# bruniss/multi-task-3d-resencoder-unet

Hardware: AMD Instinct MI355X
Metric: train patches/sec (b,c,z,y,x) ResEncM 1x128^3 (higher is better)
Workload: dtype bf16; 1 GPU; cfg2: ResEncM (6 stages, feats [32, 64, 128, 256, 512, 512], blocks [1, 3, 4, 6, 6, 6]), 1-in, heads ['sheet'], patch 128x128x128, batch 2/GPU, full train step (fwd+loss+bwd+allreduce+clip+AdamW); global_batch=2, parallelism=dp1

## Files before the change

multi-task-3d-resencoder-unet_amd/csrc/build.py:

```python
import os
import subprocess
import sys

HERE = os.path.dirname(os.path.abspath(__file__))
SOURCES = ["rx_runtime.hip", "rx_instnorm.hip", "rx_head.hip", "rx_stem.hip", "rx_pack_optim.hip", "rx_igemm.hip", "rx_wgrad.hip", "rx_wgrad_halo.hip", "rx_conv_halo.hip", "rx_stem_wgrad.hip", "rx_loss.hip", "rx_se.hip", "rx_dgrad_s2.hip", "rx_prog.hip", "rx_pointwise.hip", "rx_infer.hip", "rx_augment.hip", "rx_geometry.hip"]
HEADERS = ["rx_common.h", "rx_internal.h", "rx_reduce.h", "rx_prog.h", os.path.join("..", "..", "include", "rxunet.h")]
LIB = os.path.join(HERE, "librxunet.so")
HIPCC = os.environ.get("HIPCC", "/opt/rocm/bin/hipcc")
FLAGS = ["-O3", "--offload-arch=gfx950", "-std=c++17", "-fPIC", "-Wno-unused-result"]


def _stale(target, deps):
    if not os.path.exists(target):
        return True
    t = os.path.getmtime(target)
    return any(os.path.getmtime(d) > t for d in deps)


def build(force=False, verbose=True):
    hdrs = [os.path.join(HERE, h) for h in HEADERS] + [os.path.abspath(__file__)]
    objs = []
    procs = []
    for src in SOURCES:
        obj = os.path.join(HERE, src.replace(".hip", ".o"))
        objs.append(obj)
        if force or _stale(obj, [os.path.join(HERE, src)] + hdrs):
            cmd = [HIPCC] + FLAGS + ["-c", os.path.join(HERE, src), "-o", obj]
            if verbose:
                print(" ".join(cmd), flush=True)
            procs.append((src, subprocess.Popen(cmd, cwd=HERE)))
    for src, p in procs:
        if p.wait() != 0:
            raise RuntimeError(f"hipcc failed on {src}")
    if force or procs or _stale(LIB, objs):
        cmd = [HIPCC, "--offload-arch=gfx950", "-shared", "-fPIC", "-o", LIB] + objs
        if verbose:
            print(" ".join(cmd), flush=True)
        subprocess.check_call(cmd, cwd=HERE)
    return LIB


if __name__ == "__main__":
    print(build(force="--force" in sys.argv))
```

multi-task-3d-resencoder-unet_amd/csrc/rx_internal.h:

```cpp
#pragma once
#include "rx_common.h"

int rx_note_seq(void);

int rx_conv_halo_try(rx_dtype dt, const rx_act* in, const void* w, const float* bias, const rx_act* out, int flip, int accumulate,
                     hipStream_t st, float* stat_part, size_t stat_bytes, int* stat_chunks, const RxBwdStat* bs);
int rx_pointwise_try(rx_dtype dt, const rx_act* in, const void* w, const float* bias, const rx_act* out, const int32_t stride[3],
                     int accumulate, hipStream_t st);
int rx_dgrad_s2_halo_try(rx_dtype dt, const rx_act* dy, const void* w_bwd, const rx_act* dx, int accumulate, hipStream_t st);

size_t rx_wgrad_halo_ws_bytes(const rx_act* x, const rx_act* dy);
int rx_wgrad_halo_try(rx_dtype dt, const rx_act* x, const rx_act* dy, const int32_t stride[3], float* dw, void* ws, size_t ws_bytes,
                      hipStream_t st);
void rx_wgrad_reduce_launch(const float* slab, int S, int T_, int R, int C, float* dw, hipStream_t st);

int rx_stem_fwd_mfma_try(rx_dtype dt, const float* x, int n, int cin, int z, int y, int xx, const float* w, const float* bias,
                         const rx_act* out, const int32_t kernel[3], hipStream_t st, float* stat_part, size_t stat_bytes, int* stat_chunks);
int rx_stem_wgrad_mfma_try(rx_dtype dt, const float* x, int n, int cin, int z, int y, int xx, const rx_act* dy, const int32_t kernel[3],
                           float* partial, int max_blocks, int* nblocks_out, hipStream_t st);

void rx_colreduce_finalize_launch(hipStream_t st, const float* partial, int N, int nchunks, int nacc, int C, double V, float eps, int mode,
                                  float* out);
void rx_stats_finalize_launch(const float* partial, int N, int nchunks, int C, double V, float eps, float* stats, hipStream_t st);
void rx_inbwd_fused_finalize_launch(const float* partial, int N, int nchunks, int C, double V, const float* stats, float* m12, hipStream_t st);
```

multi-task-3d-resencoder-unet_amd/csrc/rx_wgrad.hip:

```cpp
#include <stdlib.h>

#include "rx_common.h"
#include "rx_internal.h"


struct WgradGeom {
  int Qz, Qy, Qx, Vq, NQ;
  int R, ldg;
  long g_ss;
  int Zx, Yx, Xx, Cc, ldx;
  long x_ss;
  int isz, isy, isx;
  int ntaps, ksplit, q_per_split, tiles_c;
  RxTap taps[RX_MAX_TAPS];
};


typedef __attribute__((address_space(3))) s16x4 lds_s16x4;

template <typename T>
__device__ inline u32x4 fetch_frag(const T* panel, int ks, int lane) {
  if constexpr (sizeof(T) == 2) {
    const int g16 = lane >> 4, half = g16 & 1, h = g16 >> 1, l15 = lane & 15, q4 = l15 >> 2, p4 = l15 & 3;
    const T* a0 = panel + (ks * 16 + 8 * h + q4) * 32 + 16 * half + 4 * p4;
    s16x4 t0 = __builtin_amdgcn_ds_read_tr16_b64_v4i16((lds_s16x4*)(a0));
    s16x4 t1 = __builtin_amdgcn_ds_read_tr16_b64_v4i16((lds_s16x4*)(a0 + 4 * 32));
    u32x2 lo = __builtin_bit_cast(u32x2, t0), hi = __builtin_bit_cast(u32x2, t1);
    return u32x4{lo[0], lo[1], hi[0], hi[1]};
  } else {
    const int i = lane & 31, h = lane >> 5;
    const T* a0 = panel + (ks * 8 + 4 * h) * 32 + i;
    f32x4 v = {a0[0], a0[32], a0[64], a0[96]};
    return __builtin_bit_cast(u32x4, v);
  }
}

template <typename T, int BR, int BC>
__global__ __launch_bounds__(256) void wgrad_kernel(const T* __restrict__ gt, const T* __restrict__ xt, float* __restrict__ slab,
                                                    const WgradGeom g) {
  constexpr int P = Elem<T>::PER16;
  constexpr int NR = BR / 32, NC = BC / 32;
  constexpr int GV = 64 * BR / P / 256;
  constexpr int XV = 64 * BC / P / 256;
  constexpr int KSTEPS = sizeof(T) == 2 ? 4 : 8;
  constexpr int TILE_ELEMS = 64 * (BR + BC);
  extern __shared__ __attribute__((aligned(16))) unsigned char smem[];
  T* sbuf = reinterpret_cast<T*>(smem);

  const int tid = threadIdx.x, lane = tid & 63, wave = tid >> 6;
  const int tile_r = blockIdx.x / g.tiles_c, tile_c = blockIdx.x - tile_r * g.tiles_c;
  const int r0 = tile_r * BR, c0 = tile_c * BC;
  const RxTap tp = g.taps[blockIdx.y];
  const int q_begin = blockIdx.z * g.q_per_split;
  const int q_end = min(g.NQ, q_begin + g.q_per_split);

  u32x4 gr[GV], xr[XV];
  auto load_tile = [&](int q0) {
#pragma unroll
    for (int j = 0; j < GV; ++j) {
      const int i = tid + 256 * j, vox = i / (BR / P), cv = i - vox * (BR / P);
      const int q = q0 + vox;
      u32x4 v = u32x4{0u, 0u, 0u, 0u};
      if (q < q_end) {
        const int n = q / g.Vq, vq = q - n * g.Vq;
        v = *reinterpret_cast<const u32x4*>(gt + n * g.g_ss + (long)vq * g.ldg + r0 + cv * P);
      }
      gr[j] = v;
    }
#pragma unroll
    for (int j = 0; j < XV; ++j) {
      const int i = tid + 256 * j, vox = i / (BC / P), cv = i - vox * (BC / P);
      const int q = q0 + vox;
      u32x4 v = u32x4{0u, 0u, 0u, 0u};
      if (q < q_end) {
        const int n = q / g.Vq, vq = q - n * g.Vq;
        const int qx = vq % g.Qx, t = vq / g.Qx;
        const int qy = t % g.Qy, qz = t / g.Qy;
        const int z = qz * g.isz + tp.dz, y = qy * g.isy + tp.dy, x = qx * g.isx + tp.dx;
        if ((unsigned)z < (unsigned)g.Zx && (unsigned)y < (unsigned)g.Yx && (unsigned)x < (unsigned)g.Xx)
          v = *reinterpret_cast<const u32x4*>(xt + n * g.x_ss + ((long)(z * g.Yx + y) * g.Xx + x) * g.ldx + c0 + cv * P);
      }
      xr[j] = v;
    }
  };
  auto store_tile = [&](int buf) {
    T* base = sbuf + buf * TILE_ELEMS;
#pragma unroll
    for (int j = 0; j < GV; ++j) {
      const int i = tid + 256 * j, vox = i / (BR / P), cv = i - vox * (BR / P);
      const int c = cv * P;
      *reinterpret_cast<u32x4*>(base + ((c >> 5) * 64 + vox) * 32 + (c & 31)) = gr[j];
    }
    T* xb = base + 64 * BR;
#pragma unroll
    for (int j = 0; j < XV; ++j) {
      const int i = tid + 256 * j, vox = i / (BC / P), cv = i - vox * (BC / P);
      const int c = cv * P;
      *reinterpret_cast<u32x4*>(xb + ((c >> 5) * 64 + vox) * 32 + (c & 31)) = xr[j];
    }
  };

  f32x16 acc[NR][NC];
#pragma unroll
  for (int a = 0; a < NR; ++a)
#pragma unroll
    for (int b = 0; b < NC; ++b)
#pragma unroll
      for (int r = 0; r < 16; ++r) acc[a][b][r] = 0.f;

  if (q_begin < q_end) {
    load_tile(q_begin);
    store_tile(0);
  }
  __syncthreads();
  int it = 0;
  for (int q0 = q_begin; q0 < q_end; q0 += 64, ++it) {
    const int buf = it & 1;
    if (q0 + 64 < q_end) load_tile(q0 + 64);
    const T* base = sbuf + buf * TILE_ELEMS;
#pragma unroll
    for (int kk = 0; kk < KSTEPS / 4; ++kk) {
      const int ks = wave + 4 * kk;
      u32x4 af[NR], bf[NC];
#pragma unroll
      for (int a = 0; a < NR; ++a) af[a] = fetch_frag<T>(base + a * 64 * 32, ks, lane);
#pragma unroll
      for (int b = 0; b < NC; ++b) bf[b] = fetch_frag<T>(base + 64 * BR + b * 64 * 32, ks, lane);
#pragma unroll
      for (int a = 0; a < NR; ++a)
#pragma unroll
        for (int b = 0; b < NC; ++b) Mma<T>::run(acc[a][b], af[a], bf[b]);
    }
    if (q0 + 64 < q_end) store_tile(buf ^ 1);
    __syncthreads();
  }

  float* red = reinterpret_cast<float*>(smem);
  const int col = lane & 31, fh = lane >> 5;
#pragma unroll
  for (int a = 0; a < NR; ++a)
#pragma unroll
    for (int b = 0; b < NC; ++b)
#pragma unroll
      for (int r = 0; r < 16; ++r) {
        const int row = (r & 3) + 8 * (r >> 2) + 4 * fh;
        red[(((wave * NR + a) * NC + b) * 32 + row) * 32 + col] = acc[a][b][r];
      }
  __syncthreads();
  float* out = slab + ((long)blockIdx.z * g.ntaps + blockIdx.y) * g.R * g.Cc;
  for (int i = tid; i < NR * NC * 1024; i += 256) {
    const int blk = i >> 10, rc = i & 1023, row = rc >> 5, cc = rc & 31;
    const int a = blk / NC, b = blk - a * NC;
    float s = red[i] + red[i + NR * NC * 1024] + red[i + 2 * NR * NC * 1024] + red[i + 3 * NR * NC * 1024];
    out[(long)(r0 + a * 32 + row) * g.Cc + c0 + b * 32 + cc] = s;
  }
}

__global__ __launch_bounds__(256) void wgrad_reduce(const float* __restrict__ slab, int S, int T_, int R, int C, float* __restrict__ dw) {
  __shared__ float tile[27 * 257];
  const long RC = (long)R * C;
  const long base = (long)blockIdx.x * 256;
  const long i = base + threadIdx.x;
  for (int t = 0; t < T_; ++t) {
    float s = 0.f;
    if (i < RC)
      for (int k = 0; k < S; ++k) s += slab[((long)k * T_ + t) * RC + i];
    tile[t * 257 + threadIdx.x] = s;
  }
  __syncthreads();
  const long n_here = (RC - base < 256 ? RC - base : 256) * T_;
  for (long j = threadIdx.x; j < n_here; j += 256) {
    int pair = (int)(j / T_), t = (int)(j - (long)pair * T_);
    dw[base * T_ + j] = tile[t * 257 + pair];
  }
}

__global__ __launch_bounds__(256) void wgrad_reduce_manysplits(const float* __restrict__ slab, int S, int T_, int R, int C,
                                                               float* __restrict__ dw) {
  const long RC = (long)R * C;
  const long i = (long)blockIdx.x * 256 + threadIdx.x;
  const int t = blockIdx.y;
  if (i >= RC) return;
  const float* p = slab + (long)t * RC + i;
  const long stride = (long)T_ * RC;
  float a0 = 0.f, a1 = 0.f, a2 = 0.f, a3 = 0.f, a4 = 0.f, a5 = 0.f, a6 = 0.f, a7 = 0.f;
  int k = 0;
  for (; k + 8 <= S; k += 8) {
    a0 += p[(k + 0) * stride];
    a1 += p[(k + 1) * stride];
    a2 += p[(k + 2) * stride];
    a3 += p[(k + 3) * stride];
    a4 += p[(k + 4) * stride];
    a5 += p[(k + 5) * stride];
    a6 += p[(k + 6) * stride];
    a7 += p[(k + 7) * stride];
  }
  for (; k < S; ++k) a0 += p[k * stride];
  dw[i * T_ + t] = ((a0 + a1) + (a2 + a3)) + ((a4 + a5) + (a6 + a7));
}

static int plan_split(const WgradGeom& g, int BR, int BC, size_t ws_bytes, int* ksplit, int* qps) {
  const long tiles = (long)(g.R / BR) * (g.Cc / BC) * g.ntaps;
  const long ktiles = ((long)g.NQ + 63) / 64;
  long S = (1024 + tiles - 1) / tiles;
  if (S > ktiles / 4) S = ktiles / 4;
  if (S < 1) S = 1;
  const size_t slab1 = (size_t)g.ntaps * g.R * g.Cc * sizeof(float);
  while (S > 1 && S * slab1 > ws_bytes) --S;
  if (slab1 > ws_bytes) return RX_EWORKSPACE;
  long per = (ktiles + S - 1) / S;
  S = (ktiles + per - 1) / per;
  *ksplit = (int)S;
  *qps = (int)(per * 64);
  return RX_OK;
}

static size_t wgrad_ws_bytes(int R, int C, int taps, long NQ) {
  const size_t slab1 = (size_t)taps * R * C * sizeof(float);
  const long tiles = (long)((R + 63) / 64) * ((C + 63) / 64) * taps;
  long S = (1024 + tiles - 1) / tiles;
  long ktiles = (NQ + 63) / 64;
  if (S > ktiles / 4) S = ktiles / 4;
  if (S < 1) S = 1;
  if (R % 64 || C % 64) {
    const long t32 = (long)(R / 32) * (C / 32) * taps;
    long S2 = (1024 + t32 - 1) / t32;
    if (S2 > S) S = S2;
  }
  return S * slab1 + 256;
}

template <typename T>
static void wgrad_dispatch(int BR, int BC, dim3 grid, hipStream_t st, const void* gt, const void* xt, float* slab, const WgradGeom& g) {
  const size_t lds = 65536;
#define RX_WG(BR_, BC_)                                                                                                            \
  do {                                                                                                                             \
    (void)hipFuncSetAttribute(reinterpret_cast<const void*>(&wgrad_kernel<T, BR_, BC_>), hipFuncAttributeMaxDynamicSharedMemorySize, \
                              (int)lds);                                                                                           \
    hipLaunchKernelGGL((wgrad_kernel<T, BR_, BC_>), grid, dim3(256), lds, st, (const T*)gt, (const T*)xt, slab, g);                \
  } while (0)
  if (BR == 64 && BC == 64)
    RX_WG(64, 64);
  else if (BR == 64 && BC == 32)
    RX_WG(64, 32);
  else if (BR == 32 && BC == 64)
    RX_WG(32, 64);
  else
    RX_WG(32, 32);
#undef RX_WG
}

static int wgrad_launch(rx_dtype dt, const void* gt, const void* xt, float* dw, WgradGeom& g, void* ws, size_t ws_bytes, hipStream_t st) {
  const int per16 = dt == RX_F32 ? 4 : 8;
  if (g.R % 32 || g.Cc % 32) RX_FAIL(RX_EUNSUPPORTED, "wgrad: channel counts must be multiples of 32 (R=%d C=%d)", g.R, g.Cc);
  if (g.ldg % per16 || g.ldx % per16 || ((uintptr_t)gt & 15) || ((uintptr_t)xt & 15)) RX_FAIL(RX_EUNSUPPORTED, "wgrad: misaligned operand");
  if (!ws || !dw) RX_FAIL(RX_EINVAL, "wgrad: null workspace / output");
  const int BR = g.R % 64 == 0 ? 64 : 32, BC = g.Cc % 64 == 0 ? 64 : 32;
  g.tiles_c = g.Cc / BC;
  int rc = plan_split(g, BR, BC, ws_bytes, &g.ksplit, &g.q_per_split);
  if (rc) RX_FAIL(rc, "wgrad: workspace too small (%zu bytes)", ws_bytes);
  dim3 grid((g.R / BR) * (g.Cc / BC), g.ntaps, g.ksplit);
  rx_note_kernel(BR == 64 ? (BC == 64 ? "wgrad_kernel<64,64>" : "wgrad_kernel<64,32>") : (BC == 64 ? "wgrad_kernel<32,64>" : "wgrad_kernel<32,32>"));
  RX_DISPATCH_DTYPE(dt, T, wgrad_dispatch<T>(BR, BC, grid, st, gt, xt, (float*)ws, g));
  rx_wgrad_reduce_launch((const float*)ws, g.ksplit, g.ntaps, g.R, g.Cc, dw, st);
  RX_CHECK_LAUNCH("wgrad");
  return RX_OK;
}

static int conv_out_dim(int in, int k, int s) { return (in + 2 * ((k - 1) / 2) - k) / s + 1; }

void rx_wgrad_reduce_launch(const float* slab, int S, int T_, int R, int C, float* dw, hipStream_t st) {
  long RC = (long)R * C;
  if (S >= 8 || T_ > 27)
    hipLaunchKernelGGL(wgrad_reduce_manysplits, dim3((unsigned)((RC + 255) / 256), T_), dim3(256), 0, st, slab, S, T_, R, C, dw);
  else
    hipLaunchKernelGGL(wgrad_reduce, dim3((unsigned)((RC + 255) / 256)), dim3(256), 0, st, slab, S, T_, R, C, dw);
}

extern "C" size_t rx_conv3d_bwd_weight_workspace(const rx_act* x, const rx_act* dy, const int32_t kernel[3]) {
  if (!rx_act_ok_planar(x) || !rx_act_ok(dy)) return 0;
  size_t a = wgrad_ws_bytes(dy->c, x->c, kernel[0] * kernel[1] * kernel[2], (long)dy->n * rx_act_voxels(dy));
  size_t b = (kernel[0] == 3 && kernel[1] == 3 && kernel[2] == 3) ? rx_wgrad_halo_ws_bytes(x, dy) : 0;
  return a > b ? a : b;
}

extern "C" int rx_conv3d_bwd_weight(rx_dtype dt, const rx_act* x, const rx_act* dy, float* dw, const int32_t kernel[3],
                                    const int32_t stride[3], void* ws, size_t ws_bytes, void* stream) {
  RX_RECORD(stream, [=, x_ = RxActV(x), dy_ = RxActV(dy), kernel_ = RxI3V(kernel), stride_ = RxI3V(stride)](void* s) { return rx_conv3d_bwd_weight(dt, x_.p(), dy_.p(), dw, kernel_.v, stride_.v, ws, ws_bytes, s); });
  if (!rx_act_ok_planar(x) || !rx_act_ok(dy)) RX_FAIL(RX_EINVAL, "rx_conv3d_bwd_weight: bad arguments");
  for (int i = 0; i < 3; ++i) {
    if (kernel[i] < 1 || kernel[i] > RX_MAX_KERNEL) RX_FAIL(RX_EUNSUPPORTED, "rx_conv3d_bwd_weight: kernel sizes must be 1..%d per axis", RX_MAX_KERNEL);
    if (stride[i] < 1 || stride[i] > RX_MAX_STRIDE) RX_FAIL(RX_EUNSUPPORTED, "rx_conv3d_bwd_weight: strides must be 1..%d per axis", RX_MAX_STRIDE);
  }
  if (dy->n != x->n || dy->z != conv_out_dim(x->z, kernel[0], stride[0]) || dy->y != conv_out_dim(x->y, kernel[1], stride[1]) ||
      dy->x != conv_out_dim(x->x, kernel[2], stride[2]))
    RX_FAIL(RX_EINVAL, "rx_conv3d_bwd_weight: geometry mismatch");
  if (kernel[0] == 3 && kernel[1] == 3 && kernel[2] == 3 && ws && dw) {
    int rc = rx_wgrad_halo_try(dt, x, dy, stride, dw, ws, ws_bytes, (hipStream_t)stream);
    if (rc < 0) return rc;
    if (rc == 1) return RX_OK;
  }
  if (x->cs) RX_FAIL(RX_EUNSUPPORTED, "rx_conv3d_bwd_weight: a planar-concat x needs the LDS-halo weight-gradient kernels");
  WgradGeom g;
  memset(&g, 0, sizeof(g));
  g.Qz = dy->z, g.Qy = dy->y, g.Qx = dy->x, g.Vq = (int)rx_act_voxels(dy), g.NQ = dy->n * g.Vq;
  g.R = dy->c, g.ldg = dy->ld, g.g_ss = (long)g.Vq * dy->ld;
  g.Zx = x->z, g.Yx = x->y, g.Xx = x->x, g.Cc = x->c, g.ldx = x->ld, g.x_ss = rx_act_voxels(x) * (long)x->ld;
  g.isz = stride[0], g.isy = stride[1], g.isx = stride[2];
  const int pz = (kernel[0] - 1) / 2, py = (kernel[1] - 1) / 2, px = (kernel[2] - 1) / 2;
  for (int a = 0; a < kernel[0]; ++a)
    for (int b = 0; b < kernel[1]; ++b)
      for (int c = 0; c < kernel[2]; ++c) {
        RxTap& t = g.taps[g.ntaps];
        t.dz = (int8_t)(a - pz), t.dy = (int8_t)(b - py), t.dx = (int8_t)(c - px);
        t.w = (uint16_t)g.ntaps;
        ++g.ntaps;
      }
  return wgrad_launch(dt, dy->ptr, x->ptr, dw, g, ws, ws_bytes, (hipStream_t)stream);
}

struct ConvTWgGeom {
  int Vq, NQ, Qy, Qx;
  int R, ldr;
  long r_ss;
  int Yf, Xf, Cc, ldc;
  long c_ss;
  int sz, sy, sx, ntaps;
  int q_per_split;
};

template <typename T, int NR, int NC>
__global__ __launch_bounds__(512) void convT_wgrad_kernel(const T* __restrict__ xt, const T* __restrict__ yt, float* __restrict__ slab,
                                                          const ConvTWgGeom g) {
  constexpr int P = Elem<T>::PER16;
  constexpr int BR = 32 * NR, BC = 32 * NC;
  constexpr int XV = (64 * BR / P + 511) / 512;
  constexpr int YV = (64 * BC / P + 511) / 512;
  extern __shared__ __attribute__((aligned(16))) unsigned char smem[];
  T* sX = reinterpret_cast<T*>(smem);
  T* sY = sX + 64 * BR;
  const int tid = threadIdx.x, lane = tid & 63;
  const int wave = __builtin_amdgcn_readfirstlane(tid >> 6);
  const int q_begin = blockIdx.x * g.q_per_split;
  const int q_end = min(g.NQ, q_begin + g.q_per_split);

  u32x4 xr[XV], yr[8][YV];
  auto load_tile = [&](int q0) {
#pragma unroll
    for (int j = 0; j < XV; ++j) {
      const int i = tid + 512 * j, vox = i / (BR / P), cv = i - vox * (BR / P);
      const int q = q0 + vox;
      u32x4 v = u32x4{0u, 0u, 0u, 0u};
      if (vox < 64 && q < q_end) {
        const int n = q / g.Vq, vq = q - n * g.Vq;
        v = *reinterpret_cast<const u32x4*>(xt + n * g.r_ss + (long)vq * g.ldr + cv * P);
      }
      xr[j] = v;
    }
#pragma unroll
    for (int j = 0; j < YV; ++j) {
      const int i = tid + 512 * j, vox = i / (BC / P), cv = i - vox * (BC / P);
      const int q = q0 + vox;
      const bool ok = vox < 64 && q < q_end;
      const int n = ok ? q / g.Vq : 0, vq = ok ? q - n * g.Vq : 0;
      const int qx = vq % g.Qx, t2 = vq / g.Qx;
      const int qy = t2 % g.Qy, qz = t2 / g.Qy;
      const T* base = yt + n * g.c_ss + cv * P;
#pragma unroll
      for (int t = 0; t < 8; ++t) {
        u32x4 v = u32x4{0u, 0u, 0u, 0u};
        if (ok && t < g.ntaps) {
          const int c = t % g.sx, b = (t / g.sx) % g.sy, a = t / (g.sx * g.sy);
          const long fv = ((long)(qz * g.sz + a) * g.Yf + (qy * g.sy + b)) * g.Xf + (qx * g.sx + c);
          v = *reinterpret_cast<const u32x4*>(base + fv * g.ldc);
        }
        yr[t][j] = v;
      }
    }
  };
  auto store_tile = [&]() {
#pragma unroll
    for (int j = 0; j < XV; ++j) {
      const int i = tid + 512 * j, vox = i / (BR / P), cv = i - vox * (BR / P);
      const int c = cv * P;
      if (vox < 64) *reinterpret_cast<u32x4*>(sX + ((c >> 5) * 64 + vox) * 32 + (c & 31)) = xr[j];
    }
#pragma unroll
    for (int j = 0; j < YV; ++j) {
      const int i = tid + 512 * j, vox = i / (BC / P), cv = i - vox * (BC / P);
      const int c = cv * P;
      if (vox < 64) {
#pragma unroll
        for (int t = 0; t < 8; ++t)
          if (t < g.ntaps) *reinterpret_cast<u32x4*>(sY + (long)t * 64 * BC + ((c >> 5) * 64 + vox) * 32 + (c & 31)) = yr[t][j];
      }
    }
  };

  f32x16 acc[NR][NC];
#pragma unroll
  for (int a = 0; a < NR; ++a)
#pragma unroll
    for (int b = 0; b < NC; ++b)
#pragma unroll
      for (int r = 0; r < 16; ++r) acc[a][b][r] = 0.f;

  if (q_begin < q_end) load_tile(q_begin);
  for (int q0 = q_begin; q0 < q_end; q0 += 64) {
    __syncthreads();
    store_tile();
    __syncthreads();
    if (q0 + 64 < q_end) load_tile(q0 + 64);
    if (wave < g.ntaps) {
      const T* yb = sY + (long)wave * 64 * BC;
#pragma unroll
      for (int ks = 0; ks < 4; ++ks) {
        u32x4 af[NR], bf[NC];
#pragma unroll
        for (int a = 0; a < NR; ++a) af[a] = fetch_frag<T>(sX + a * 64 * 32, ks, lane);
#pragma unroll
        for (int b = 0; b < NC; ++b) bf[b] = fetch_frag<T>(yb + b * 64 * 32, ks, lane);
#pragma unroll
        for (int a = 0; a < NR; ++a)
#pragma unroll
          for (int b = 0; b < NC; ++b) Mma<T>::run(acc[a][b], af[a], bf[b]);
      }
    }
  }
  if (wave < g.ntaps) {
    const int col = lane & 31, fh = lane >> 5;
    float* out = slab + ((long)blockIdx.x * g.ntaps + wave) * g.R * g.Cc;
#pragma unroll
    for (int a = 0; a < NR; ++a)
#pragma unroll
      for (int b = 0; b < NC; ++b)
#pragma unroll
        for (int r = 0; r < 16; ++r) {
          const int row = (r & 3) + 8 * (r >> 2) + 4 * fh;
          out[(long)(a * 32 + row) * g.Cc + b * 32 + col] = acc[a][b][r];
        }
  }
}

static int convT_wgrad_splits(long NQ, size_t slab1) {
  long ktiles = (NQ + 63) / 64;
  long S = ktiles / 8;
  if (S > 256) S = 256;
  while (S > 32 && (size_t)S * slab1 > ((size_t)32 << 20)) S /= 2;
  if (S < 1) S = 1;
  return (int)S;
}

static int convT_wgrad_try(rx_dtype dt, const rx_act* x, const rx_act* dy, const int32_t stride[3], float* dw, void* ws, size_t ws_bytes,
                           hipStream_t st) {
  const int taps = stride[0] * stride[1] * stride[2];
  const int R = x->c, C = dy->c;
  if (dt == RX_F32 || taps > 8 || R % 32 || C % 32 || x->ld % 8 || dy->ld % 8 || ((uintptr_t)x->ptr & 15) || ((uintptr_t)dy->ptr & 15)) return 0;
  const int NR = R / 32, NC = C / 32;
  if (!((NR == 2 && NC == 1) || (NR == 4 && NC == 2) || (NR == 1 && NC == 1) || (NR == 2 && NC == 2))) return 0;
  const long NQ = (long)x->n * rx_act_voxels(x);
  if (NQ < 32768) return 0;
  const size_t slab1 = (size_t)taps * R * C * sizeof(float);
  const int S = convT_wgrad_splits(NQ, slab1);
  if ((size_t)S * slab1 > ws_bytes) return 0;
  ConvTWgGeom g;
  g.Vq = (int)rx_act_voxels(x), g.NQ = (int)NQ, g.Qy = x->y, g.Qx = x->x;
  g.R = R, g.ldr = x->ld, g.r_ss = (long)g.Vq * x->ld;
  g.Yf = dy->y, g.Xf = dy->x, g.Cc = C, g.ldc = dy->ld, g.c_ss = rx_act_voxels(dy) * (long)dy->ld;
  g.sz = stride[0], g.sy = stride[1], g.sx = stride[2], g.ntaps = taps;
  const long ktiles = (NQ + 63) / 64;
  g.q_per_split = (int)(((ktiles + S - 1) / S) * 64);
  const int S2 = (int)((NQ + g.q_per_split - 1) / g.q_per_split);
  const size_t lds = (size_t)64 * (R + taps * C) * 2;
  rx_note_kernel("convT_wgrad_kernel");
#define RX_CTW(NR_, NC_)                                                                                                              \
  do {                                                                                                                                \
    (void)hipFuncSetAttribute(reinterpret_cast<const void*>(&convT_wgrad_kernel<T, NR_, NC_>), hipFuncAttributeMaxDynamicSharedMemorySize, 160 * 1024); \
    hipLaunchKernelGGL((convT_wgrad_kernel<T, NR_, NC_>), dim3(S2), dim3(512), lds, st, (const T*)x->ptr, (const T*)dy->ptr, (float*)ws, g);            \
  } while (0)
#define RX_CTW_ALL()                       \
  if (NR == 2 && NC == 1) RX_CTW(2, 1);    \
  else if (NR == 4 && NC == 2) RX_CTW(4, 2); \
  else if (NR == 1 && NC == 1) RX_CTW(1, 1); \
  else RX_CTW(2, 2)
  if (dt == RX_BF16) {
    using T = bf16_t;
    RX_CTW_ALL();
  } else {
    using T = f16_t;
    RX_CTW_ALL();
  }
#undef RX_CTW_ALL
#undef RX_CTW
  rx_wgrad_reduce_launch((const float*)ws, S2, taps, R, C, dw, st);
  return 1;
}

extern "C" size_t rx_convT3d_bwd_weight_workspace(const rx_act* x, const rx_act* dy, const int32_t stride[3]) {
  if (!rx_act_ok(x) || !rx_act_ok(dy)) return 0;
  const int taps = stride[0] * stride[1] * stride[2];
  const long NQ = (long)x->n * rx_act_voxels(x);
  const size_t slab1 = (size_t)taps * x->c * dy->c * sizeof(float);
  const size_t a = wgrad_ws_bytes(x->c, dy->c, taps, NQ);
  const size_t b = (size_t)convT_wgrad_splits(NQ, slab1) * slab1 + 256;
  return a > b ? a : b;
}

extern "C" int rx_convT3d_bwd_weight(rx_dtype dt, const rx_act* x, const rx_act* dy, float* dw, const int32_t stride[3], void* ws,
                                     size_t ws_bytes, void* stream) {
  RX_RECORD(stream, [=, x_ = RxActV(x), dy_ = RxActV(dy), stride_ = RxI3V(stride)](void* s) { return rx_convT3d_bwd_weight(dt, x_.p(), dy_.p(), dw, stride_.v, ws, ws_bytes, s); });
  if (!rx_act_ok(x) || !rx_act_ok(dy)) RX_FAIL(RX_EINVAL, "rx_convT3d_bwd_weight: bad arguments");
  for (int i = 0; i < 3; ++i)
    if (stride[i] < 1 || stride[i] > RX_MAX_STRIDE) RX_FAIL(RX_EUNSUPPORTED, "rx_convT3d_bwd_weight: strides must be 1..%d per axis", RX_MAX_STRIDE);
  if (dy->n != x->n || dy->z != x->z * stride[0] || dy->y != x->y * stride[1] || dy->x != x->x * stride[2])
    RX_FAIL(RX_EINVAL, "rx_convT3d_bwd_weight: geometry mismatch");
  if (ws && dw) {
    const int rc = convT_wgrad_try(dt, x, dy, stride, dw, ws, ws_bytes, (hipStream_t)stream);
    if (rc < 0) return rc;
    if (rc == 1) {
      RX_CHECK_LAUNCH("rx_convT3d_bwd_weight(convT_wgrad)");
      return RX_OK;
    }
  }
  WgradGeom g;
  memset(&g, 0, sizeof(g));
  g.Qz = x->z, g.Qy = x->y, g.Qx = x->x, g.Vq = (int)rx_act_voxels(x), g.NQ = x->n * g.Vq;
  g.R = x->c, g.ldg = x->ld, g.g_ss = (long)g.Vq * x->ld;
  g.Zx = dy->z, g.Yx = dy->y, g.Xx = dy->x, g.Cc = dy->c, g.ldx = dy->ld, g.x_ss = rx_act_voxels(dy) * (long)dy->ld;
  g.isz = stride[0], g.isy = stride[1], g.isx = stride[2];
  for (int a = 0; a < stride[0]; ++a)
    for (int b = 0; b < stride[1]; ++b)
      for (int c = 0; c < stride[2]; ++c) {
        RxTap& t = g.taps[g.ntaps];
        t.dz = (int8_t)a, t.dy = (int8_t)b, t.dx = (int8_t)c;
        t.w = (uint16_t)g.ntaps;
        ++g.ntaps;
      }
  return wgrad_launch(dt, x->ptr, dy->ptr, dw, g, ws, ws_bytes, (hipStream_t)stream);
}
```

Before: 118.4 patches/s.

## Add dedicated stride-2 3x3x3 weight-gradient kernel with parity-plane LDS tiling

Adds a new MFMA weight-gradient kernel for stride-2 3x3x3 convolutions. It stages the input halo in LDS as eight parity sub-planes so each tap reads contiguous transposed fragments. Tiles are double-buffered via buffer-load-to-LDS, work is split across output tiles, and partial slabs are reduced afterwards. It is tried before the generic halo path, meant to cut the cost of the strided downsampling convs in backward, at the price of extra code and workspace-dependent split counts.

```diff
diff --git a/multi-task-3d-resencoder-unet_amd/csrc/build.py b/multi-task-3d-resencoder-unet_amd/csrc/build.py
--- a/multi-task-3d-resencoder-unet_amd/csrc/build.py
+++ b/multi-task-3d-resencoder-unet_amd/csrc/build.py
@@ -3,7 +3,7 @@
 import sys
 
 HERE = os.path.dirname(os.path.abspath(__file__))
-SOURCES = ["rx_runtime.hip", "rx_instnorm.hip", "rx_head.hip", "rx_stem.hip", "rx_pack_optim.hip", "rx_igemm.hip", "rx_wgrad.hip", "rx_wgrad_halo.hip", "rx_conv_halo.hip", "rx_stem_wgrad.hip", "rx_loss.hip", "rx_se.hip", "rx_dgrad_s2.hip", "rx_prog.hip", "rx_pointwise.hip", "rx_infer.hip", "rx_augment.hip", "rx_geometry.hip"]
+SOURCES = ["rx_runtime.hip", "rx_instnorm.hip", "rx_head.hip", "rx_stem.hip", "rx_pack_optim.hip", "rx_igemm.hip", "rx_wgrad.hip", "rx_wgrad_halo.hip", "rx_wgrad_s2.hip", "rx_conv_halo.hip", "rx_stem_wgrad.hip", "rx_loss.hip", "rx_se.hip", "rx_dgrad_s2.hip", "rx_prog.hip", "rx_pointwise.hip", "rx_infer.hip", "rx_augment.hip", "rx_geometry.hip"]
 HEADERS = ["rx_common.h", "rx_internal.h", "rx_reduce.h", "rx_prog.h", os.path.join("..", "..", "include", "rxunet.h")]
 LIB = os.path.join(HERE, "librxunet.so")
 HIPCC = os.environ.get("HIPCC", "/opt/rocm/bin/hipcc")
diff --git a/multi-task-3d-resencoder-unet_amd/csrc/rx_internal.h b/multi-task-3d-resencoder-unet_amd/csrc/rx_internal.h
--- a/multi-task-3d-resencoder-unet_amd/csrc/rx_internal.h
+++ b/multi-task-3d-resencoder-unet_amd/csrc/rx_internal.h
@@ -12,6 +12,8 @@
 size_t rx_wgrad_halo_ws_bytes(const rx_act* x, const rx_act* dy);
 int rx_wgrad_halo_try(rx_dtype dt, const rx_act* x, const rx_act* dy, const int32_t stride[3], float* dw, void* ws, size_t ws_bytes,
                       hipStream_t st);
+int rx_wgrad_s2_try(rx_dtype dt, const rx_act* x, const rx_act* dy, const int32_t stride[3], float* dw, void* ws, size_t ws_bytes,
+                    hipStream_t st);
 void rx_wgrad_reduce_launch(const float* slab, int S, int T_, int R, int C, float* dw, hipStream_t st);
 
 int rx_stem_fwd_mfma_try(rx_dtype dt, const float* x, int n, int cin, int z, int y, int xx, const float* w, const float* bias,
diff --git a/multi-task-3d-resencoder-unet_amd/csrc/rx_wgrad.hip b/multi-task-3d-resencoder-unet_amd/csrc/rx_wgrad.hip
--- a/multi-task-3d-resencoder-unet_amd/csrc/rx_wgrad.hip
+++ b/multi-task-3d-resencoder-unet_amd/csrc/rx_wgrad.hip
@@ -296,7 +296,8 @@
       dy->x != conv_out_dim(x->x, kernel[2], stride[2]))
     RX_FAIL(RX_EINVAL, "rx_conv3d_bwd_weight: geometry mismatch");
   if (kernel[0] == 3 && kernel[1] == 3 && kernel[2] == 3 && ws && dw) {
-    int rc = rx_wgrad_halo_try(dt, x, dy, stride, dw, ws, ws_bytes, (hipStream_t)stream);
+    int rc = rx_wgrad_s2_try(dt, x, dy, stride, dw, ws, ws_bytes, (hipStream_t)stream);
+    if (rc == 0) rc = rx_wgrad_halo_try(dt, x, dy, stride, dw, ws, ws_bytes, (hipStream_t)stream);
     if (rc < 0) return rc;
     if (rc == 1) return RX_OK;
   }
diff --git a/multi-task-3d-resencoder-unet_amd/csrc/rx_wgrad_s2.hip b/multi-task-3d-resencoder-unet_amd/csrc/rx_wgrad_s2.hip
--- /dev/null
+++ b/multi-task-3d-resencoder-unet_amd/csrc/rx_wgrad_s2.hip
@@ -0,0 +1,248 @@
+#include <stdlib.h>
+
+#include <type_traits>
+
+#include "rx_common.h"
+#include "rx_internal.h"
+
+namespace {
+
+struct WgS2Geom {
+  int N, Z, Y, X;
+  int Zi, Yi, Xi;
+  int R, Cc, ldg, ldx;
+  long g_ss, x_ss;
+  int tz_n, ty_n, tx_n, NT;
+  int S, tiles_per_split, panels_c;
+};
+
+constexpr int S2_TZ = 2, S2_TY = 4, S2_TX = 8;
+constexpr int s2_pl_nz(int p) { return S2_TZ + (p >> 2); }
+constexpr int s2_pl_ny(int p) { return S2_TY + ((p >> 1) & 1); }
+constexpr int s2_pl_nx(int p) { return S2_TX + (p & 1); }
+constexpr int s2_pl_base(int p) {
+  int b = 0;
+  for (int q = 0; q < p; ++q) b += s2_pl_nz(q) * s2_pl_ny(q) * s2_pl_nx(q);
+  return b;
+}
+constexpr int S2_HV = s2_pl_base(8);
+constexpr int S2_XINSTR = (S2_HV + 15) / 16;
+constexpr int S2_XPIECES = S2_XINSTR / 8;
+static_assert(S2_HV == 765 && S2_XINSTR == 48, "2x4x8 tile");
+constexpr int s2_buf_bytes(int NR) { return (64 * NR + 16 * S2_XINSTR) * 64; }
+
+constexpr int s2_xoff(int s, int t) {
+  const int kz = t / 9, ky = (t / 3) % 3, kx = t % 3;
+  const int p = (kz != 1) * 4 + (ky != 1) * 2 + (kx != 1);
+  const int oz = kz == 2, oy = ky == 2, ox = kx == 2;
+  return (s2_pl_base(p) + (((s >> 1) + oz) * s2_pl_ny(p) + 2 * (s & 1) + oy) * s2_pl_nx(p) + ox) * 64;
+}
+
+typedef __attribute__((address_space(3))) s16x4 lds_s16x4_s2;
+typedef __attribute__((address_space(3))) unsigned char lds_byte_s2;
+
+__device__ inline u32x4 s2_tr_frag(const lds_byte_s2* p, int off0, int off1) {
+  s16x4 t0 = __builtin_amdgcn_ds_read_tr16_b64_v4i16((lds_s16x4_s2*)(p + off0));
+  s16x4 t1 = __builtin_amdgcn_ds_read_tr16_b64_v4i16((lds_s16x4_s2*)(p + off1));
+  u32x2 lo = __builtin_bit_cast(u32x2, t0), hi = __builtin_bit_cast(u32x2, t1);
+  return u32x4{lo[0], lo[1], hi[0], hi[1]};
+}
+
+template <typename T, int NG, int W>
+__device__ __forceinline__ void s2_tile_mma(const lds_byte_s2* gb, const lds_byte_s2* xb0, const lds_byte_s2* xb1,
+                                            f32x16 (&acc)[(27 + NG - 1) / NG]) {
+  constexpr int NJ = (27 - W + NG - 1) / NG;
+  u32x4 fa[2], fb[NJ];
+  auto read_a = [&](int s) { return s2_tr_frag(gb, s * 1024, s * 1024 + 256); };
+  auto read_b = [&](int s, int j) {
+    const int t = W + NG * j;
+    const int off = s2_xoff(s, t);
+    return s2_tr_frag((t % 3) != 1 ? xb1 : xb0, off, off + 256);
+  };
+  fa[0] = read_a(0);
+#pragma unroll
+  for (int j = 0; j < NJ; ++j) fb[j] = read_b(0, j);
+#pragma unroll
+  for (int s = 0; s < 4; ++s) {
+    if (s + 1 < 4) fa[(s + 1) & 1] = read_a(s + 1);
+    __builtin_amdgcn_sched_barrier(0);
+#pragma unroll
+    for (int j = 0; j < NJ; ++j) {
+      Mma<T>::run(acc[j], fa[s & 1], fb[j]);
+      if (s + 1 < 4) fb[j] = read_b(s + 1, j);
+      __builtin_amdgcn_sched_barrier(0);
+    }
+  }
+}
+
+template <typename T, int NR>
+__global__ __launch_bounds__(512, 1) void wgrad_s2pp_kernel(const T* __restrict__ gt, const T* __restrict__ xt, float* __restrict__ slab,
+                                                            const WgS2Geom g) {
+  constexpr int NG = NR == 2 ? 4 : 8, MAXJ = (27 + NG - 1) / NG;
+  constexpr int BUF = s2_buf_bytes(NR), XOFF = 64 * NR * 64;
+  extern __shared__ __attribute__((aligned(16))) unsigned char smem[];
+  const int tid = threadIdx.x, lane = tid & 63;
+  const int wave = __builtin_amdgcn_readfirstlane(tid >> 6);
+  const int PPn = gridDim.x, lid = rx_xcd_remap(blockIdx.y * PPn + blockIdx.x, PPn * gridDim.y);
+  const int split = lid / PPn, pp = lid - split * PPn;
+  const int pr = pp / g.panels_c, pc = pp - pr * g.panels_c;
+  const int r0 = pr * 32 * NR, c0 = pc * 32;
+  const int t_begin = split * g.tiles_per_split;
+  const int t_end = min(g.NT, t_begin + g.tiles_per_split);
+
+  const int chunk = lane & 3, lrow = lane >> 2;
+  int xh[S2_XPIECES];
+#pragma unroll
+  for (int p = 0; p < S2_XPIECES; ++p) {
+    const int row = 16 * (wave + 8 * p) + lrow;
+    int v = -1;
+#pragma unroll
+    for (int q = 0; q < 8; ++q) {
+      const int l = row - s2_pl_base(q);
+      if (l >= 0 && l < s2_pl_nz(q) * s2_pl_ny(q) * s2_pl_nx(q)) {
+        const int ix = l % s2_pl_nx(q), r2 = l / s2_pl_nx(q);
+        const int iy = r2 % s2_pl_ny(q), iz = r2 / s2_pl_ny(q);
+        v = ((2 * iz + 1 - (q >> 2)) << 16) | ((2 * iy + 1 - ((q >> 1) & 1)) << 8) | (2 * ix + 1 - (q & 1));
+      }
+    }
+    xh[p] = v;
+  }
+  const unsigned OOB = 0x7fffff00u;
+  const long gbytes = (long)g.N * g.g_ss * 2, xbytes = (long)g.N * g.x_ss * 2;
+  __amdgpu_buffer_rsrc_t rG = __builtin_amdgcn_make_buffer_rsrc((void*)gt, 0, (unsigned)(gbytes > 0xfffffff0L ? 0xfffffff0L : gbytes), 0x00020000);
+  __amdgpu_buffer_rsrc_t rX = __builtin_amdgcn_make_buffer_rsrc((void*)xt, 0, (unsigned)(xbytes > 0xfffffff0L ? 0xfffffff0L : xbytes), 0x00020000);
+  auto dma_tile = [&](int tile, int buf) {
+    int tx, ty, tz, n;
+    rx_tile_coords(tile, g.tx_n, g.ty_n, g.tz_n, 1, n, tz, ty, tx);
+    const int z0 = tz * S2_TZ, y0 = ty * S2_TY, x0 = tx * S2_TX;
+    lds_byte_s2* lG = (lds_byte_s2*)(smem + buf * BUF);
+    lds_byte_s2* lX = lG + XOFF;
+    if (wave < 4 * NR) {
+      const int v = 16 * wave + lrow, a = v >> 6, lv = v & 63;
+      const int z = z0 + (lv >> 5), y = y0 + ((lv >> 3) & 3), x = x0 + (lv & 7);
+      const unsigned gbase = (unsigned)((n * g.g_ss + r0 + a * 32 + chunk * 8) * 2);
+      const unsigned off = (z < g.Z && y < g.Y && x < g.X) ? gbase + (unsigned)(((z * g.Y + y) * g.X + x) * g.ldg * 2) : OOB;
+      __builtin_amdgcn_raw_ptr_buffer_load_lds(rG, (__attribute__((address_space(3))) void*)(lG + 1024 * wave), 16, off, 0, 0, 0);
+    }
+    const unsigned xbase = (unsigned)((n * g.x_ss + c0 + chunk * 8) * 2);
+    const int zb = 2 * z0 - 1, yb = 2 * y0 - 1, xb = 2 * x0 - 1;
+#pragma unroll
+    for (int p = 0; p < S2_XPIECES; ++p) {
+      if (xh[p] >= 0) {
+        const int z = zb + (xh[p] >> 16), y = yb + ((xh[p] >> 8) & 255), x = xb + (xh[p] & 255);
+        const bool ok = (unsigned)z < (unsigned)g.Zi && (unsigned)y < (unsigned)g.Yi && (unsigned)x < (unsigned)g.Xi;
+        const unsigned off = ok ? xbase + (unsigned)(((z * g.Yi + y) * g.Xi + x) * g.ldx * 2) : OOB;
+        __builtin_amdgcn_raw_ptr_buffer_load_lds(rX, (__attribute__((address_space(3))) void*)(lX + 1024 * (wave + 8 * p)), 16, off, 0, 0, 0);
+      }
+    }
+  };
+
+  const int g16 = lane >> 4, half = g16 & 1, h = g16 >> 1, l15 = lane & 15, q4 = l15 >> 2, p4 = l15 & 3;
+  const int colb = (16 * half + 4 * p4) * 2;
+  const int pa = wave / NG;
+  const int g_off = pa * 4096 + (8 * h + q4) * 64 + colb;
+  const int x0_off = XOFF + (h * S2_TX + q4) * 64 + colb;
+  const int x1_off = XOFF + (h * (S2_TX + 1) + q4) * 64 + colb;
+
+  f32x16 acc[MAXJ];
+#pragma unroll
+  for (int j = 0; j < MAXJ; ++j)
+#pragma unroll
+    for (int r = 0; r < 16; ++r) acc[j][r] = 0.f;
+
+  auto run = [&](auto wc) {
+    constexpr int W = decltype(wc)::value;
+    if (t_begin < t_end) dma_tile(t_begin, 0);
+    asm volatile("s_waitcnt vmcnt(0)" ::: "memory");
+    __syncthreads();
+    for (int tile = t_begin; tile < t_end; ++tile) {
+      const int buf = (tile - t_begin) & 1;
+      if (tile + 1 < t_end) dma_tile(tile + 1, buf ^ 1);
+      const lds_byte_s2* base = (const lds_byte_s2*)(smem) + buf * BUF;
+      s2_tile_mma<T, NG, W>(base + g_off, base + x0_off, base + x1_off, acc);
+      asm volatile("s_waitcnt vmcnt(0)" ::: "memory");
+      __syncthreads();
+    }
+  };
+  switch (wave % NG) {
+    case 0: run(std::integral_constant<int, 0>{}); break;
+    case 1: run(std::integral_constant<int, 1>{}); break;
+    case 2: run(std::integral_constant<int, 2>{}); break;
+    case 3: run(std::integral_constant<int, 3>{}); break;
+    case 4: run(std::integral_constant<int, 4 % NG>{}); break;
+    case 5: run(std::integral_constant<int, 5 % NG>{}); break;
+    case 6: run(std::integral_constant<int, 6 % NG>{}); break;
+    default: run(std::integral_constant<int, 7 % NG>{}); break;
+  }
+
+  const int col = lane & 31, fh = lane >> 5, W = wave % NG;
+#pragma unroll
+  for (int j = 0; j < MAXJ; ++j) {
+    const int t = W + NG * j;
+    if (t < 27) {
+      float* out = slab + (((long)split * 27 + t) * g.R + r0 + 32 * pa) * g.Cc + c0;
+#pragma unroll
+      for (int r = 0; r < 16; ++r) {
+        const int row = (r & 3) + 8 * (r >> 2) + 4 * fh;
+        out[(long)row * g.Cc + col] = acc[j][r];
+      }
+    }
+  }
+}
+
+template <typename T, int NR>
+void s2_launch(dim3 grid, hipStream_t st, const rx_act* dy, const rx_act* x, void* ws, const WgS2Geom& g) {
+  const int lds = 2 * s2_buf_bytes(NR);
+  (void)hipFuncSetAttribute(reinterpret_cast<const void*>(&wgrad_s2pp_kernel<T, NR>), hipFuncAttributeMaxDynamicSharedMemorySize, lds);
+  hipLaunchKernelGGL((wgrad_s2pp_kernel<T, NR>), grid, dim3(512), lds, st, (const T*)dy->ptr, (const T*)x->ptr, (float*)ws, g);
+}
+
+}
+
+#define RX_WGS2_MIN_TILES 64
+#define RX_WGS2_CUS 256
+
+int rx_wgrad_s2_try(rx_dtype dt, const rx_act* x, const rx_act* dy, const int32_t stride[3], float* dw, void* ws, size_t ws_bytes,
+                    hipStream_t st) {
+  if (dt == RX_F32 || stride[0] != 2 || stride[1] != 2 || stride[2] != 2 || x->cs) return 0;
+  if (x->z != 2 * dy->z || x->y != 2 * dy->y || x->x != 2 * dy->x) return 0;
+  if (x->c % 32 || dy->c % 32 || x->ld % 8 || dy->ld % 8 || ((uintptr_t)x->ptr & 15) || ((uintptr_t)dy->ptr & 15)) return 0;
+  WgS2Geom g;
+  memset(&g, 0, sizeof(g));
+  g.N = dy->n, g.Z = dy->z, g.Y = dy->y, g.X = dy->x;
+  g.Zi = x->z, g.Yi = x->y, g.Xi = x->x;
+  g.R = dy->c, g.Cc = x->c, g.ldg = dy->ld, g.ldx = x->ld;
+  g.g_ss = rx_act_voxels(dy) * (long)dy->ld;
+  g.x_ss = rx_act_voxels(x) * (long)x->ld;
+  if ((long)g.N * g.g_ss * 2 >= 0x7fffff00L || (long)g.N * g.x_ss * 2 >= 0x7fffff00L) return 0;
+  const int NR = g.R % 64 == 0 ? 2 : 1;
+  g.tz_n = (g.Z + S2_TZ - 1) / S2_TZ, g.ty_n = (g.Y + S2_TY - 1) / S2_TY, g.tx_n = (g.X + S2_TX - 1) / S2_TX;
+  const long NT = (long)g.N * g.tz_n * g.ty_n * g.tx_n;
+  g.panels_c = g.Cc / 32;
+  const long PPn = (long)(g.R / (32 * NR)) * g.panels_c;
+  if (NT < RX_WGS2_MIN_TILES || NT * PPn < RX_WGS2_CUS || NT > 0x3fffffffL || PPn > 65535) return 0;
+  g.NT = (int)NT;
+  long S = (RX_WGS2_CUS + PPn - 1) / PPn;
+  if (S > NT) S = NT;
+  const size_t slab1 = (size_t)27 * g.R * g.Cc * sizeof(float);
+  while (S > 1 && S * slab1 > ws_bytes) --S;
+  if (slab1 > ws_bytes) return 0;
+  g.tiles_per_split = (int)((NT + S - 1) / S);
+  g.S = (g.NT + g.tiles_per_split - 1) / g.tiles_per_split;
+  dim3 grid((unsigned)PPn, g.S);
+  rx_note_kernel("wgrad_s2pp_kernel");
+  if (dt == RX_BF16) {
+    if (NR == 2) s2_launch<bf16_t, 2>(grid, st, dy, x, ws, g);
+    else s2_launch<bf16_t, 1>(grid, st, dy, x, ws, g);
+  } else {
+    if (NR == 2) s2_launch<f16_t, 2>(grid, st, dy, x, ws, g);
+    else s2_launch<f16_t, 1>(grid, st, dy, x, ws, g);
+  }
+  rx_wgrad_reduce_launch((const float*)ws, g.S, 27, g.R, g.Cc, dw, st);
+  hipError_t e = hipGetLastError();
+  if (e != hipSuccess) {
+    rx_set_error("wgrad_s2pp: %s", hipGetErrorString(e));
+    return RX_ELAUNCH;
+  }
+  return 1;
+}
```

Result: no change. 118.8 patches/s (median of 6 runs) (+0.4%).
